# google-deepmind/bsuite

Hardware: AMD Instinct MI355X
Metric: env-steps/sec (higher is better)
Workload: dtype int32; 1 GPU; deep_sea/10 deep_sea {'size': 30, 'mapping_seed': 42} random actions, dense TimeStep; mode=e, lanes_per_gpu=1048576, global_lanes=1048576, episode_phases=staggered

## Files before the change

bsuite_amd/csrc/bsx_pair_device.h:

```cpp
#ifndef BSX_PAIR_DEVICE_H_
#define BSX_PAIR_DEVICE_H_

#include "bsx_device.h"
#include "bsx_policy.h"

template <class Fam, bool LEAN, bool NOMT>
__device__ __forceinline__ int bsx_fam_advance(const typename Fam::args& a, const typename Fam::shared& s, int64_t i, uint64_t lane,
                                               uint64_t step, int32_t st, int act, int32_t& nst, double& reward) {
  return Fam::template advance_nomt<LEAN, NOMT>(a, s, i, lane, step, st, act, nst, reward);
}

template <class Fam, bool LEAN = false, int MT = -1, int LPT = 1>
__device__ __forceinline__ void bsx_advance_body(const typename Fam::args& a, uint32_t block_id,
                                                 typename Fam::shared& s_fam, unsigned int* s_cnt,
                                                 int32_t* s_state = nullptr) {
  if (threadIdx.x < 2) s_cnt[threadIdx.x] = 0;
  Fam::stage(a, s_fam);
  __syncthreads();
  if constexpr (LPT == 2) {
    const uint64_t step = bsx_step_of(a.ctl);
    int64_t i[2];
    bool mine[2];
    int act[2], type[2] = {-1, -1};
    int32_t st[2];
// ... 145 lines not shown
      }
    }
  }
  if (mine) a.state[i] = st;
  bsx_pool_counts(a.ctl, n_last, n_first, s_cnt, block_id & (BSX_COUNTER_SHARDS - 1));
}

struct bsx_policy_args {
  const uint8_t* table;
  const int32_t* policy_index;
  int32_t* actions_out;
  double epsilon;
  uint64_t explore_seed;
  int32_t n_states, n_policies;
  uint32_t num_actions;
  int32_t in_lds;
};

template <class Fam, class HotFn>
__global__ void __launch_bounds__(BSX_BLOCK) bsx_policy_rollout_kernel(const typename Fam::args a, const int n_steps,
                                                                             int32_t* __restrict__ rows, const HotFn fn,
                                                                             const bsx_policy_args p) {
  __shared__ typename Fam::shared s_fam;
  __shared__ unsigned int s_cnt[2];
  __shared__ uint8_t s_tab[BSX_POLICY_LDS_BYTES];
  if (threadIdx.x < 2) s_cnt[threadIdx.x] = 0;
  Fam::stage(a, s_fam);
  const int S = p.n_states;
  const bool in_lds = p.in_lds != 0;
  if (in_lds) {
    for (int k = threadIdx.x; k < S; k += BSX_BLOCK) s_tab[k] = p.table[k];
  }
  __syncthreads();
  const int64_t B = a.ctl.n_lanes;
  const int64_t i = (int64_t)blockIdx.x * BSX_BLOCK + threadIdx.x;
  const bool mine = i < B;
  const uint64_t lane = a.ctl.lane_offset + (uint64_t)i;
  const uint64_t step0 = bsx_step_of(a.ctl);
  const bool explore = p.epsilon > 0.0;
  int32_t st = mine ? a.state[i] : 0;
  const uint8_t* __restrict__ tab = p.table;
  if (mine && p.policy_index != nullptr) tab += (int64_t)bsx_policy_clamp(p.policy_index[i], p.n_policies) * S;
  uint32_t n_last = 0, n_first = 0;
  uint32_t block_id = blockIdx.x;
#if defined(__HIP_DEVICE_COMPILE__)
  asm volatile("" : "+v"(block_id));
#endif
  if (mine) {
#pragma unroll 1
    for (int t = 0; t < n_steps; ++t) {
      const uint64_t step = step0 + (uint64_t)t;
      const int64_t oi = (int64_t)t * B + i;
      const int key = bsx_policy_clamp(fn.policy_key(st), S);
      uint32_t entry;
      if (in_lds) {
        entry = s_tab[key];
#if defined(__HIP_DEVICE_COMPILE__)
        asm volatile("" : "+v"(entry));
#endif
      } else {
        entry = tab[key];
      }
      uint32_t w0 = 0, w1 = 0, w2 = 0;
      if (explore) {
        const bsx_u32x4 w = bsx_policy_draws(p.explore_seed, lane, step);
        w0 = w.v[0]; w1 = w.v[1]; w2 = w.v[2];
      }
      const int act = bsx_policy_select(entry, Fam::resets(st), p.epsilon, w0, w1, w2, p.num_actions);
      int32_t nst; double reward;
      const int type = Fam::template advance<true>(a, s_fam, i, lane, step, st, act, nst, reward);
      st = nst;
      bsx_emit_at<0, 0, false, -1, BSX_OUT_SCALARS.rollout>(a.ctl, a.out, i, oi, lane, step, type, reward);
      bsx_index_store<BSX_OUT_INDEX.rollout>(rows, oi, nst, fn);
      bsx_st<BSX_OUT_SCALARS.rollout>(&p.actions_out[oi], (int32_t)act);
      n_last += type == BSX_LAST ? 1u : 0u;
      n_first += type == BSX_FIRST ? 1u : 0u;
    }
    a.state[i] = st;
  }
  bsx_pool_counts(a.ctl, n_last, n_first, s_cnt, block_id & (BSX_COUNTER_SHARDS - 1));
}

template <class Fam, class HotFn>
__device__ __forceinline__ void bsx_tab_eval_body(const typename Fam::args& a, const int n_steps, const HotFn& fn,
                                                  const bsx_policy_args& p, const bsx_policy_eval_t& out,
                                                  typename Fam::shared& s_fam, unsigned int* s_cnt, uint8_t* s_tab) {
  if (threadIdx.x < 2) s_cnt[threadIdx.x] = 0;
  Fam::stage(a, s_fam);
  const int S = p.n_states;
  const bool in_lds = p.in_lds != 0;
  if (in_lds) {
    for (int k = threadIdx.x; k < S; k += BSX_BLOCK) s_tab[k] = p.table[k];
  }
  __syncthreads();
  const int64_t i = (int64_t)blockIdx.x * BSX_BLOCK + threadIdx.x;
  const bool mine = i < a.ctl.n_lanes;
  const uint64_t lane = a.ctl.lane_offset + (uint64_t)i;
  const uint64_t step0 = bsx_step_of(a.ctl);
  const bool explore = p.epsilon > 0.0;
  uint32_t n_last = 0, n_first = 0;
  if (mine) {
    int32_t st = a.state[i];
    const uint8_t* __restrict__ tab = p.table;
    if (p.policy_index != nullptr) tab += (int64_t)bsx_policy_clamp(p.policy_index[i], p.n_policies) * S;
    bsx_eval_acc e = {0.0, 0.0, 0.0, 0};
    typename Fam::deferred pend = {};
#pragma unroll 1
    for (int t = 0; t < n_steps; ++t) {
      const uint64_t step = step0 + (uint64_t)t;
      const int key = bsx_policy_clamp(fn.policy_key(st), S);
      uint32_t entry;
      if (in_lds) {
        entry = s_tab[key];
#if defined(__HIP_DEVICE_COMPILE__)
        asm volatile("" : "+v"(entry));
#endif
      } else {
        entry = tab[key];
      }
      uint32_t w0 = 0, w1 = 0, w2 = 0;
      if (explore) {
        const bsx_u32x4 w = bsx_policy_draws(p.explore_seed, lane, step);
        w0 = w.v[0]; w1 = w.v[1]; w2 = w.v[2];
      }
      const int act = bsx_policy_select(entry, Fam::resets(st), p.epsilon, w0, w1, w2, p.num_actions);
      int32_t nst; double reward;
      const int type = Fam::advance_deferred(a, s_fam, i, lane, step, st, act, nst, reward, pend);
      st = nst;
      bsx_eval_accumulate(&e, type, reward);
      n_first += type == BSX_FIRST ? 1u : 0u;
    }
    n_last = (uint32_t)e.n;
    a.state[i] = st;
    out.episodes[i] = e.n;
    out.return_sum[i] = e.total;
    out.episode_return_sum[i] = e.done;
    Fam::commit_deferred(a, i, pend);
  }
  bsx_pool_counts(a.ctl, n_last, n_first, s_cnt, blockIdx.x);
}


template <class HotFn>
struct bsx_stream_seg {
  float* obs;
  const int32_t* state;
  int64_t n_lanes;
  uint32_t cells;
  uint32_t cells_magic;
  bsx_div64 dv;
  HotFn fn;
};

template <class HotFn, int K, int BS, bool NT = false>
__device__ __forceinline__ void bsx_hot_stream_body(float* __restrict__ obs,
                                                    const int32_t* __restrict__ state,
                                                    int64_t n_lanes, uint32_t cells,
                                                    uint32_t cells_magic, bsx_div64 dv,
                                                    const HotFn& fn, uint32_t block_id, int wave_contig = 1) {
  const uint64_t total = (uint64_t)n_lanes * cells;
  const uint64_t F0 = (uint64_t)block_id * (uint64_t)(K * 4 * BS);
  const uint64_t lane_b = __umul64hi(F0, dv.m) >> dv.s;
  const uint32_t r_b = (uint32_t)(F0 - lane_b * cells);
  const bool aligned = (cells & 3u) == 0;
  bsx_f4* __restrict__ o4 = reinterpret_cast<bsx_f4*>(obs + F0);
  const int32_t* __restrict__ st = state + lane_b;
  const uint64_t lanes_left = (uint64_t)n_lanes - lane_b;

  uint32_t dl[K];
  int r0[K];
  int32_t s0[K], s1[K];
  bool live[K];
#pragma unroll
  for (int u = 0; u < K; ++u) {
    const uint32_t c = wave_contig ? ((threadIdx.x >> 6) * (K * 64) + u * 64 + (threadIdx.x & 63))
                                   : (threadIdx.x + u * BS);
    const uint32_t f = r_b + (c << 2);
    dl[u] = __umulhi(f, cells_magic);
    r0[u] = (int)(f - dl[u] * cells);
    live[u] = F0 + ((uint64_t)c << 2) + 3 < total;
    s0[u] = live[u] ? st[dl[u]] : 0;
    s1[u] = (live[u] && !aligned && (uint64_t)dl[u] + 1 < lanes_left) ? st[dl[u] + 1] : 0;
  }
#pragma unroll
  for (int u = 0; u < K; ++u) {
    if (!live[u]) continue;
    int ha, hb;
    fn(s0[u], ha, hb);
    const int a0 = ha < 0 ? -1 : ha - r0[u], b0 = hb < 0 ? -1 : hb - r0[u];
    bsx_f4 v;
    v.x = (a0 == 0 || b0 == 0) ? 1.0f : 0.0f;
    v.y = (a0 == 1 || b0 == 1) ? 1.0f : 0.0f;
    v.z = (a0 == 2 || b0 == 2) ? 1.0f : 0.0f;
    v.w = (a0 == 3 || b0 == 3) ? 1.0f : 0.0f;
    const int over = (int)cells - r0[u];
    if (!aligned && over < 4) {
      int na, nb;
      fn(s1[u], na, nb);
      const int a1 = na < 0 ? -1 : na + over, b1 = nb < 0 ? -1 : nb + over;
      if (over <= 1) v.y = (a1 == 1 || b1 == 1) ? 1.0f : 0.0f;
      if (over <= 2) v.z = (a1 == 2 || b1 == 2) ? 1.0f : 0.0f;
      v.w = (a1 == 3 || b1 == 3) ? 1.0f : 0.0f;
    }
    {
      bsx_f4* dst = &o4[wave_contig ? ((threadIdx.x >> 6) * (K * 64) + u * 64 + (threadIdx.x & 63)) : (threadIdx.x + u * BS)];
      if (NT) __builtin_nontemporal_store(v, dst);
      else *dst = v;
    }
  }
  const uint64_t tail0 = total & ~3ull;
  if (tail0 != total && tail0 >= F0 && tail0 < F0 + (uint64_t)(K * 4 * BS) && threadIdx.x < 3) {
    const uint64_t F = tail0 + threadIdx.x;
    if (F < total) {
      const uint32_t f = r_b + (uint32_t)(F - F0);
      const uint32_t d = __umulhi(f, cells_magic);
      const int r = (int)(f - d * cells);
      int ha, hb;
      fn(st[d], ha, hb);
      obs[F] = (ha == r || hb == r) ? 1.0f : 0.0f;
    }
  }
}

template <class HotFn, int K, int BS>
__global__ void __launch_bounds__(BS) bsx_hot_stream_kernel(float* __restrict__ obs,
                                                                   const int32_t* __restrict__ state,
                                                                   int64_t n_lanes, uint32_t cells,
                                                                   uint32_t cells_magic, bsx_div64 dv,
                                                                   HotFn fn, int wave_contig) {
  bsx_hot_stream_body<HotFn, K, BS>(obs, state, n_lanes, cells, cells_magic, dv, fn, blockIdx.x, wave_contig);
}

template <class HotFn, int POLICY = BSX_ST_PLAIN>
__device__ __forceinline__ void bsx_tile_stream(float* __restrict__ tile, const int32_t* s_state, int lanes_here,
                                                uint32_t cells, uint32_t cells_magic, const HotFn& fn) {
  const uint32_t total = (uint32_t)lanes_here * cells;
  const uint32_t n_chunks = total >> 2;
  const bool aligned = (cells & 3u) == 0;
  bsx_f4* __restrict__ t4 = reinterpret_cast<bsx_f4*>(tile);
  for (uint32_t c = threadIdx.x; c < n_chunks; c += BSX_BLOCK) {
    const uint32_t f = c << 2;
    const uint32_t dl = bsx_div_cells(f, cells, cells_magic);
    const int r0 = (int)(f - dl * cells);
    int ha, hb;
    fn(s_state[dl], ha, hb);
    const int a0 = ha < 0 ? -1 : ha - r0, b0 = hb < 0 ? -1 : hb - r0;
    bsx_f4 v;
    v.x = (a0 == 0 || b0 == 0) ? 1.0f : 0.0f;
    v.y = (a0 == 1 || b0 == 1) ? 1.0f : 0.0f;
    v.z = (a0 == 2 || b0 == 2) ? 1.0f : 0.0f;
    v.w = (a0 == 3 || b0 == 3) ? 1.0f : 0.0f;
    const int over = (int)cells - r0;
    if (!aligned && over < 4) {
      int na, nb;
      fn(s_state[dl + 1], na, nb);
      const int a1 = na < 0 ? -1 : na + over, b1 = nb < 0 ? -1 : nb + over;
      if (over <= 1) v.y = (a1 == 1 || b1 == 1) ? 1.0f : 0.0f;
      if (over <= 2) v.z = (a1 == 2 || b1 == 2) ? 1.0f : 0.0f;
      v.w = (a1 == 3 || b1 == 3) ? 1.0f : 0.0f;
    }
    bsx_st<POLICY>(&t4[c], v);
  }
  const uint32_t f = (n_chunks << 2) + threadIdx.x;
  if (threadIdx.x < 3 && f < total) {
    const uint32_t dl = bsx_div_cells(f, cells, cells_magic);
    const int r = (int)(f - dl * cells);
    int ha, hb;
    fn(s_state[dl], ha, hb);
    tile[f] = (ha == r || hb == r) ? 1.0f : 0.0f;
  }
}

template <class Fam, bool LEAN, class HotFn>
__global__ void __launch_bounds__(BSX_BLOCK) bsx_fused_tile_kernel(const typename Fam::args a, float* __restrict__ obs,
                                                                   const uint32_t cells, const uint32_t cells_magic,
                                                                   const HotFn fn) {
  __shared__ typename Fam::shared s_fam;
  __shared__ unsigned int s_cnt[2];
  __shared__ int32_t s_state[BSX_BLOCK];
  bsx_advance_body<Fam, LEAN>(a, blockIdx.x, s_fam, s_cnt, s_state);
  const int64_t lane0 = (int64_t)blockIdx.x * BSX_BLOCK;
  const int64_t left = a.ctl.n_lanes - lane0;
  bsx_tile_stream<HotFn, BSX_ST_WT>(obs + lane0 * (int64_t)cells, s_state, left < BSX_BLOCK ? (int)left : BSX_BLOCK, cells, cells_magic, fn);
}

template <class Fam, bool LEAN, class HotFn>
__global__ void __launch_bounds__(BSX_BLOCK) bsx_fused_tile64_kernel(const typename Fam::args a, float* __restrict__ obs,
                                                                     const uint32_t cells, const uint32_t cells_magic,
                                                                     const HotFn fn) {
  __shared__ typename Fam::shared s_fam;
  __shared__ int32_t s_state[BSX_WAVE];
  Fam::stage(a, s_fam);
  __syncthreads();
  const int64_t lane0 = (int64_t)blockIdx.x * BSX_WAVE;
  const int64_t i = lane0 + threadIdx.x;
  int type = -1;
  if (threadIdx.x < BSX_WAVE && i < a.ctl.n_lanes) {
    const uint64_t lane = a.ctl.lane_offset + (uint64_t)i;
    const uint64_t step = bsx_step_of(a.ctl);
    int32_t nst; double reward;
    const int act = a.ctl.force_reset ? 0 : bsx_action(a.ctl, a.action, i, step);
    const int32_t st = a.ctl.state_in != nullptr ? a.ctl.state_in[i] : a.state[i];
    type = Fam::template advance<LEAN>(a, s_fam, i, lane, step, st, act, nst, reward);
    a.state[i] = nst;
    s_state[threadIdx.x] = nst;
    if (LEAN) bsx_emit_at<0, 0, false>(a.ctl, a.out, i, i, lane, step, type, reward);
    else bsx_emit(a.ctl, a.out, i, lane, step, type, reward);
  }
  if (threadIdx.x < BSX_WAVE && a.ctl.counters != nullptr) {
    const unsigned long long last = __ballot(type == BSX_LAST), first = __ballot(type == BSX_FIRST);
    if (threadIdx.x == 0 && (last | first) != 0ull) {
      unsigned long long* shard = (unsigned long long*)a.ctl.counters + (size_t)(blockIdx.x & (BSX_COUNTER_SHARDS - 1)) * BSX_COUNTER_STRIDE;
      if (last) atomicAdd(&shard[0], (unsigned long long)__popcll(last));
      if (first) atomicAdd(&shard[1], (unsigned long long)__popcll(first));
    }
  }
  __syncthreads();
  const int64_t left = a.ctl.n_lanes - lane0;
  bsx_tile_stream<HotFn, BSX_ST_WT>(obs + lane0 * (int64_t)cells, s_state, left < BSX_WAVE ? (int)left : BSX_WAVE, cells, cells_magic, fn);
}

template <class Fam, bool LEAN, class HotFn>
__global__ void __launch_bounds__(BSX_BLOCK) bsx_fused_rollout_kernel(const typename Fam::args a, const int n_steps,
                                                                      float* __restrict__ obs, const uint32_t cells,
                                                                      const uint32_t cells_magic, const HotFn fn) {
  __shared__ typename Fam::shared s_fam;
  __shared__ unsigned int s_cnt[2];
  __shared__ int32_t s_state[2][BSX_BLOCK];
  if (threadIdx.x < 2) s_cnt[threadIdx.x] = 0;
  Fam::stage(a, s_fam);
  __syncthreads();
  const int64_t B = a.ctl.n_lanes;
  const int64_t lane0 = (int64_t)blockIdx.x * BSX_BLOCK;
  const int64_t i = lane0 + threadIdx.x;
  const bool mine = i < B;
  const int lanes_here = B - lane0 < BSX_BLOCK ? (int)(B - lane0) : BSX_BLOCK;
  const uint64_t lane = a.ctl.lane_offset + (uint64_t)i;
  const uint64_t step0 = bsx_step_of(a.ctl);
  int32_t st = mine ? a.state[i] : 0;
  int act_next = mine ? a.action[i] : 0;
#pragma unroll 1
  for (int t = 0; t < n_steps; ++t) {
    int type = -1;
    const int act = act_next;
    if (mine) {
      if (t + 1 < n_steps) act_next = a.action[(int64_t)(t + 1) * B + i];
      int32_t nst; double reward;
      type = Fam::template advance<LEAN>(a, s_fam, i, lane, step0 + (uint64_t)t, st, act, nst, reward);
      st = nst;
      s_state[t & 1][threadIdx.x] = nst;
      if (LEAN) bsx_emit_at<0, 0, false>(a.ctl, a.out, i, (int64_t)t * B + i, lane, step0 + (uint64_t)t, type, reward);
      else bsx_emit_at(a.ctl, a.out, i, (int64_t)t * B + i, lane, step0 + (uint64_t)t, type, reward);
    }
    bsx_count_types(a.ctl, type, s_cnt);
    __syncthreads();
    bsx_tile_stream<HotFn, BSX_ST_NT>(obs + ((int64_t)t * B + lane0) * (int64_t)cells, s_state[t & 1], lanes_here, cells, cells_magic, fn);
  }
  if (mine) a.state[i] = st;
  bsx_final_barrier();
  bsx_flush_counts(a.ctl, s_cnt, blockIdx.x);
}

template <class Fam, bool LEAN, class HotFn, int K>
__global__ void __launch_bounds__(BSX_BLOCK) bsx_pipelined_kernel(const typename Fam::args a, const uint32_t adv_blocks,
// ... 163 lines not shown
```

bsuite_amd/csrc/bsx_pair_host.h:

```cpp
#ifndef BSX_PAIR_HOST_H_
#define BSX_PAIR_HOST_H_

#include "bsx_host.h"
#include "bsx_pair_device.h"

template <class Fam>
static inline int bsx_launch_advance(const typename Fam::args& a, hipStream_t st) {
  const int64_t blocks = bsx_blocks_of(a.ctl.n_lanes);
  if (blocks > 0x7FFFFFFF) return BSX_EINVAL;
  const bool lean = bsx_ctl_lean(a.ctl);
  static const int lpt2_min_blocks = bsx_env_int("BSX_ADVANCE_LPT2_MIN_BLOCKS", 4096);
  if (lean && lpt2_min_blocks > 0 && blocks >= lpt2_min_blocks) {
    bsx_advance2_kernel<Fam><<<dim3((unsigned)((blocks + 1) / 2)), dim3(BSX_BLOCK), 0, st>>>(a);
    return 0;
  }
  if (lean) bsx_advance_kernel<Fam, true><<<dim3((unsigned)blocks), dim3(BSX_BLOCK), 0, st>>>(a);
  else if (a.ctl.mt_state == nullptr) bsx_advance_kernel<Fam, false, 0><<<dim3((unsigned)blocks), dim3(BSX_BLOCK), 0, st>>>(a);
  else bsx_advance_kernel<Fam, false><<<dim3((unsigned)blocks), dim3(BSX_BLOCK), 0, st>>>(a);
  return 0;
}

void bsx_launch_pair_advance_delta(int32_t family, const void* args, const void* fn, int32_t* paint, uint32_t cells, int64_t blocks,
                                   hipStream_t st);

template <class Fam, class HotFn>
static inline int bsx_launch_advance_delta(const typename Fam::args& a, const HotFn& fn, int32_t* paint,
                                           uint32_t cells, hipStream_t st) {
  const int64_t blocks = bsx_blocks_of(a.ctl.n_lanes);
  if (blocks > 0x7FFFFFFF) return BSX_EINVAL;
  bsx_launch_pair_advance_delta(HotFn::FAMILY, &a, &fn, paint, cells, blocks, st);
  return 0;
}

int bsx_launch_hot_cells(float* obs, const int32_t* state, int64_t n_lanes, uint32_t cells, int32_t family, int32_t p0, int32_t p1,
                         hipStream_t st);

template <class HotFn, int K>
static inline int bsx_launch_hot_stream(float* obs, const int32_t* state, int64_t n_lanes, uint32_t cells,
                                        uint32_t cells_magic, HotFn fn, hipStream_t st) {
  const uint64_t total = (uint64_t)n_lanes * cells;
  if (cells < 4u || (reinterpret_cast<uintptr_t>(obs) & 15u) != 0)
    return bsx_launch_hot_cells(obs, state, n_lanes, cells, HotFn::FAMILY, fn.geom0(), fn.geom1(), st);
  const bsx_div64 dv = bsx_make_div64(cells);
  const uint64_t per_block = (uint64_t)K * 4 * BSX_BLOCK;
  const uint64_t blocks = (total + per_block - 1) / per_block;
  if (blocks > 0x7FFFFFFFull) return BSX_EINVAL;
  bsx_hot_stream_kernel<HotFn, K, BSX_BLOCK><<<dim3((unsigned)blocks), dim3(BSX_BLOCK), 0, st>>>(obs, state, n_lanes, cells, cells_magic, dv, fn, 1);
  return 0;
}

template <class HotFn, int K>
static inline int bsx_launch_narrow_stream(void* obs, const int32_t* state, int64_t n_lanes, uint32_t cells, int code,
                                           HotFn fn, hipStream_t st) {
  static const uint32_t one[4] = {0u, 0x01u, 0x3C00u, 0x3F80u};
  const int E = code == 1 ? 1 : 2, N = 16 / E;
  const uint64_t total = (uint64_t)n_lanes * cells;
  uint64_t head = ((16u - (reinterpret_cast<uintptr_t>(obs) & 15u)) & 15u) / (uint64_t)E;
  if (head > total) head = total;
  const uint64_t n_chunks = (total - head) / (uint64_t)N;
  const uint64_t per_block = (uint64_t)K * BSX_BLOCK;
  const uint64_t blocks = n_chunks == 0 ? 1 : (n_chunks + per_block - 1) / per_block;
  if (blocks > 0x7FFFFFFFull) return BSX_EINVAL;
  const bool wide = cells >= (uint32_t)N;
  const uint32_t magic = wide ? bsx_div_magic(cells) : 0u;
  const bsx_div64 dv = wide ? bsx_make_div64(cells) : bsx_div64{0, 0};
  const dim3 grid((unsigned)blocks), block(BSX_BLOCK);
  if (E == 1)
    bsx_narrow_stream_kernel<HotFn, 1, K><<<grid, block, 0, st>>>((uint8_t*)obs, state, n_lanes, cells, magic, dv,
                                                                   (uint32_t)head, n_chunks, one[code], fn);
  else
    bsx_narrow_stream_kernel<HotFn, 2, K><<<grid, block, 0, st>>>((uint8_t*)obs, state, n_lanes, cells, magic, dv,
                                                                   (uint32_t)head, n_chunks, one[code], fn);
  return 0;
}

template <class HotFn>
static inline bsx_stream_seg<HotFn> bsx_make_stream_seg(float* obs, const int32_t* state, int64_t n_lanes, uint32_t cells, const HotFn& fn) {
  bsx_stream_seg<HotFn> sg;
  sg.obs = obs; sg.state = state; sg.n_lanes = n_lanes; sg.cells = cells;
  sg.cells_magic = bsx_div_magic(cells); sg.dv = bsx_make_div64(cells); sg.fn = fn;
  return sg;
}

template <class Fam, class HotFn>
static inline int bsx_group_put_pair(bsx_group* g, int32_t index, const typename Fam::args& a, float* obs,
                                     int32_t* state, uint32_t cells, const HotFn& fn, int k) {
  if (cells < 4u) return BSX_ERANGE;
  memcpy(&g->args[(size_t)index * sizeof(typename Fam::args)], &a, sizeof(a));
  const bsx_stream_seg<HotFn> sg = bsx_make_stream_seg(obs, state, a.ctl.n_lanes, cells, fn);
  memcpy(&g->args2[(size_t)index * sizeof(sg)], &sg, sizeof(sg));
  const uint64_t b1 = (uint64_t)bsx_blocks_of(a.ctl.n_lanes);
  const uint64_t b2 = bsx_flat_blocks((uint64_t)a.ctl.n_lanes * cells, k);
  if (b1 > 0x3FFFFFFFull || b2 > 0x3FFFFFFFull) return BSX_EINVAL;
  g->blocks[index] = (int32_t)b1; g->blocks2[index] = (int32_t)b2;
  g->is_set[index] = 1;
  return 0;
}

void bsx_launch_pair_advance_group(int32_t family, const void* table, const bsx_group_index& gi, int64_t total_blocks, hipStream_t st);

template <class Fam, class HotFn, int K>
static int bsx_group_launch_pair(bsx_group* g, int phase, hipStream_t st) {
  if (phase != 1) bsx_launch_pair_advance_group(HotFn::FAMILY, g->d_args, g->index1(), g->total_blocks, st);
  if (phase != 0)
    bsx_hot_stream_group_kernel<HotFn, K><<<dim3((unsigned)g->total_blocks2), dim3(BSX_BLOCK), 0, st>>>(
        (const bsx_stream_seg<HotFn>*)g->d_args2, g->index2());
  return (int)hipGetLastError();
}

int bsx_launch_index_decode(int32_t* rows, const int32_t* state, int64_t n_lanes, int32_t family, int32_t p0, int32_t p1,
                            bool rollout, hipStream_t st);

static inline int bsx_check_policy_scalars(const bsx_call_t* call, const bsx_policy_t* pol, int32_t n_states) {
  if (call == nullptr || pol == nullptr) return BSX_ENULL;
  if ((call->flags & (BSX_CALL_OBS_MASK | BSX_CALL_OBS_INDEX)) != BSX_CALL_OBS_INDEX) return BSX_EMODE;
  if (call->logging != nullptr || call->wrap.kind != BSX_WRAP_NONE || call->stream.mt_state != nullptr ||
      call->stream.mt_pos != nullptr || call->reward_f64 != nullptr || call->obs_paint != nullptr ||
      call->state_alt != nullptr || call->action_ring > 1 || call->force_reset)
    return BSX_EMODE;
  if (call->n_steps < 1 || call->n_lanes < 0 || call->n_lanes > ((int64_t)1 << 40)) return BSX_EINVAL;
  if (pol->n_states != n_states || pol->n_policies < 1) return BSX_EINVAL;
  if (!(pol->epsilon >= 0.0 && pol->epsilon <= 1.0)) return BSX_ERANGE;
  return 0;
}

static inline int bsx_check_policy_call(const bsx_call_t* call, const bsx_policy_t* pol, int32_t n_states, const int32_t* state,
                                        const bsx_timestep_t& out, const double* info) {
  const int rc = bsx_check_policy_scalars(call, pol, n_states);
  if (rc != 0 || call->n_lanes == 0) return rc;
  if (pol->table == nullptr || pol->actions_out == nullptr || state == nullptr || info == nullptr ||
      out.reward == nullptr || out.discount == nullptr || out.step_type == nullptr || out.observation == nullptr)
    return BSX_ENULL;
  if (pol->n_policies > 1 && pol->policy_index == nullptr) return BSX_ENULL;
  if ((reinterpret_cast<uintptr_t>(out.observation) & 15u) != 0) return BSX_EALIGN;
  return 0;
}

static inline int bsx_check_policy_eval_call(const bsx_call_t* call, const bsx_policy_t* pol, int32_t n_states,
                                             const int32_t* state, const bsx_policy_eval_t& out, const double* info) {
  const int rc = bsx_check_policy_scalars(call, pol, n_states);
  if (rc != 0 || call->n_lanes == 0) return rc;
  if (pol->table == nullptr || state == nullptr || info == nullptr || out.episodes == nullptr || out.return_sum == nullptr ||
      out.episode_return_sum == nullptr)
    return BSX_ENULL;
  if (pol->n_policies > 1 && pol->policy_index == nullptr) return BSX_ENULL;
  if (call->action_ring < 0) return BSX_EINVAL;
  if (bsx_blocks_of(call->n_lanes) > 0x7FFFFFFF) return BSX_EINVAL;
  return 0;
}

static inline bsx_policy_args bsx_make_policy_args(const bsx_policy_t* pol, uint32_t num_actions) {
  bsx_policy_args p;
  p.table = pol->table;
  p.policy_index = pol->n_policies > 1 ? pol->policy_index : nullptr;
  p.actions_out = pol->actions_out;
  p.epsilon = pol->epsilon;
  p.explore_seed = pol->explore_seed;
  p.n_states = pol->n_states; p.n_policies = pol->n_policies;
  p.num_actions = num_actions;
  p.in_lds = (pol->n_policies == 1 && pol->n_states <= BSX_POLICY_LDS_BYTES) ? 1 : 0;
  return p;
}

template <class Fam, class HotFn>
static int bsx_policy_rollout_call(const typename Fam::args& a, const bsx_call_t* call, const bsx_policy_t* pol,
                                   uint32_t num_actions, bsx_timestep_t out, const HotFn& fn) {
// ... 122 lines not shown
```

bsuite_amd/csrc/deep_sea.hip:

```cpp
#include "bsx_pair_host.h"
#include "bsx_tab_eval.h"
#include "bsx_tab_sample_device.h"
#include "deep_sea_fam.h"
#include "pair_mixed.h"

template <int K>
__global__ void __launch_bounds__(BSX_BLOCK) deep_sea_step1_kernel(const deep_sea_fam::args a, const uint32_t cells,
                                                                   const uint32_t cells_magic, const bsx_div64 dv) {
  __shared__ deep_sea_fam::shared s_map[BSX_BLOCK / BSX_WAVE];
  const int wl = (int)(threadIdx.x & 63u);
  deep_sea_fam::shared& map = s_map[threadIdx.x >> 6];
  const int64_t n_lanes = a.ctl.n_lanes;
  const uint64_t step = bsx_step_of(a.ctl);
  const int32_t tag_new = (int32_t)(((uint32_t)(step + 1) & 1u) << DS_TAG_SHIFT);
  const bool forced = a.ctl.force_reset != 0;
  const deep_sea_hot fn{a.size};
  const uint64_t total = (uint64_t)n_lanes * cells;
  const uint64_t F0 = (uint64_t)blockIdx.x * (uint64_t)(K * 4 * BSX_BLOCK);
  const uint64_t lane_b = __umul64hi(F0, dv.m) >> dv.s;
  const uint32_t r_b = (uint32_t)(F0 - lane_b * cells);
  bsx_f4* __restrict__ o4 = reinterpret_cast<bsx_f4*>(a.out.observation + F0);
  const int32_t* __restrict__ st_b = a.state + lane_b;
  const int32_t* __restrict__ act_b = a.action + (forced ? 0 : lane_b);

  uint32_t dl[K];
  int r0[K];
  bool live[K];
#pragma unroll
  for (int u = 0; u < K; ++u) {
    const uint32_t c = (threadIdx.x >> 6) * (K * 64) + u * 64 + (threadIdx.x & 63);
    const uint32_t f = r_b + (c << 2);
    dl[u] = __umulhi(f, cells_magic);
    r0[u] = (int)(f - dl[u] * cells);
    live[u] = F0 + ((uint64_t)c << 2) + 3 < total;
  }
  const uint32_t dA = dl[0];
  uint32_t dB = dA;
  bool wrA = false, wrB = false;
#pragma unroll
  for (int u = 0; u < K; ++u) {
    if (live[u]) dB = dl[u];
  }
#pragma unroll
  for (int u = 0; u < K; ++u) {
    wrA |= live[u] && r0[u] == 0 && dl[u] == dA;
    wrB |= live[u] && r0[u] == 0 && dl[u] == dB && dB != dA;
  }
  const bool any = live[0];
  const int32_t wA = any ? st_b[dA] : 0, wB = any ? st_b[dB] : 0;
  const int aA = (any && !forced) ? act_b[dA] : 0, aB = (any && !forced) ? act_b[dB] : 0;

  const int map_words = (a.size * a.size + 31) >> 5;
  static_assert(DS_MAP_WORDS <= 2 * BSX_WAVE, "the per-wave copy of the action mapping is two passes at most");
  if (wl < map_words) map.map[wl] = a.mapping_bits[wl];
  if (wl + BSX_WAVE < map_words) map.map[wl + BSX_WAVE] = a.mapping_bits[wl + BSX_WAVE];
  bsx_wave_sync();


  auto resolve = [&](uint32_t d, int32_t w, int act, bool writer, int& type) -> int32_t {
    type = -1;
    if (!writer && (w & DS_TAG_BIT) == tag_new) return w;
    const int64_t L = (int64_t)lane_b + d;
    int32_t nst; double reward;
    const int ty = deep_sea_fam::advance<true, 1>(a, map, L, a.ctl.lane_offset + (uint64_t)L, step, w, act, nst, reward, writer);
    if (writer) {
      type = ty;
      a.state[L] = nst;
      bsx_emit_at<0, 0, false>(a.ctl, a.out, L, L, a.ctl.lane_offset + (uint64_t)L, step, ty, reward);
    }
    return nst;
  };
  int tA = -1, tB = -1;
  int32_t nA = 0, nB = 0;
  if (any) {
    nA = resolve(dA, wA, aA, wrA, tA);
    nB = dB != dA ? resolve(dB, wB, aB, wrB, tB) : nA;
  }
  int hA, hB, unused;
  fn(nA, hA, unused);
  fn(nB, hB, unused);
#pragma unroll
  for (int u = 0; u < K; ++u) {
    if (!live[u]) continue;
    int hot = dl[u] == dA ? hA : hB;
    const int p0 = hot < 0 ? -1 : hot - r0[u];
    bsx_f4 v;
    v.x = p0 == 0 ? 1.0f : 0.0f;
    v.y = p0 == 1 ? 1.0f : 0.0f;
    v.z = p0 == 2 ? 1.0f : 0.0f;
    v.w = p0 == 3 ? 1.0f : 0.0f;
    o4[(threadIdx.x >> 6) * (K * 64) + u * 64 + (threadIdx.x & 63)] = v;
  }
  const unsigned int n_last = (unsigned int)__popcll(__ballot(tA == BSX_LAST)) + (unsigned int)__popcll(__ballot(tB == BSX_LAST));
  const unsigned int n_first = (unsigned int)__popcll(__ballot(tA == BSX_FIRST)) + (unsigned int)__popcll(__ballot(tB == BSX_FIRST));
  if (a.ctl.counters != nullptr && wl == 0 && (n_last | n_first) != 0u) {
    unsigned long long* shard = (unsigned long long*)a.ctl.counters +
                                (size_t)((blockIdx.x * (BSX_BLOCK / BSX_WAVE) + (threadIdx.x >> 6)) & (BSX_COUNTER_SHARDS - 1)) * BSX_COUNTER_STRIDE;
    if (n_last) atomicAdd(&shard[0], (unsigned long long)n_last);
    if (n_first) atomicAdd(&shard[1], (unsigned long long)n_first);
  }
}

static int deep_sea_check_cfg(const bsx_deep_sea_t* cfg) {
  return (cfg->size < 1 || cfg->size > BSX_DEEP_SEA_MAX_SIZE) ? BSX_ERANGE : 0;
}

static void deep_sea_fill(const bsx_deep_sea_t* cfg, const bsx_call_t* call, const int32_t* action, int32_t* state,
                          bsx_timestep_t out, double* info, deep_sea_fam::args* a) {
  a->ctl = bsx_make_ctl(call);
  a->action = action; a->state = state; a->out = out; a->info = info;
  a->move_cost = cfg->move_cost; a->inv_size = cfg->inv_size;
  a->size = cfg->size; a->deterministic = cfg->deterministic;
  for (int w = 0; w < DS_MAP_WORDS; ++w) a->mapping_bits[w] = cfg->mapping_bits[w];
}

static int deep_sea_make(const bsx_deep_sea_t* cfg, const bsx_call_t* call, const int32_t* action,
                         int32_t* state, bsx_timestep_t out, double* info, deep_sea_fam::args* a) {
  if (cfg == nullptr) return BSX_ENULL;
  int rc = bsx_check_call(call, action, out, true, true);
  if (rc != 0) return rc;
  if ((rc = deep_sea_check_cfg(cfg)) != 0) return rc;
  if (call->stream.mt_state != nullptr && !cfg->deterministic && call->stream.mt_gauss == nullptr)
    return BSX_ENULL;
  if (call->n_lanes > 0 && (state == nullptr || info == nullptr)) return BSX_ENULL;
  deep_sea_fill(cfg, call, action, state, out, info, a);
  return 0;
}

extern "C" int bsx_deep_sea_step(const bsx_deep_sea_t* cfg, const bsx_call_t* call,
                                 const int32_t* action, int32_t* state, bsx_timestep_t out,
                                 double* info) {
  deep_sea_fam::args a;
  int rc = deep_sea_make(cfg, call, action, state, out, info, &a);
  if (rc != 0) return rc;
  if (call->n_lanes == 0) return 0;
  const uint32_t cells = (uint32_t)(cfg->size * cfg->size);
  static const int step1_env = bsx_env_int("BSX_DEEP_SEA_STEP1", 1);
  if (step1_env != 0 && (int64_t)call->n_lanes * cells * 4 <= ((int64_t)1 << 30) && (call->flags & BSX_CALL_STATE_TAGGED) && call->n_steps <= 1 && call->action_ring <= 1 && cfg->deterministic && bsx_ctl_lean(a.ctl) &&
      call->obs_paint == nullptr && bsx_call_obs(call) == 0 && !bsx_call_index(call) && (cells & 3u) == 0 && cells >= 3u * 256u) {
    constexpr int K = 4;
    const uint64_t total = (uint64_t)call->n_lanes * cells;
    const uint64_t blocks = (total + (uint64_t)K * 4 * BSX_BLOCK - 1) / ((uint64_t)K * 4 * BSX_BLOCK);
    if (blocks > 0x7FFFFFFFull) return BSX_EINVAL;
    deep_sea_step1_kernel<K><<<dim3((unsigned)blocks), dim3(BSX_BLOCK), 0, (hipStream_t)call->hip_stream>>>(
        a, cells, bsx_div_magic(cells), bsx_make_div64(cells));
    return bsx_launch_status();
  }
  return bsx_pair_call<deep_sea_fam, deep_sea_hot, 4>(a, call, action, state, out, cells, deep_sea_hot{cfg->size});
}

extern "C" int bsx_deep_sea_policy_rollout(const bsx_deep_sea_t* cfg, const bsx_call_t* call, const bsx_policy_t* policy,
                                           int32_t* state, bsx_timestep_t out, double* info) {
  if (cfg == nullptr || call == nullptr || policy == nullptr) return BSX_ENULL;
  int rc = deep_sea_check_cfg(cfg);
  if (rc == 0) rc = bsx_check_policy_call(call, policy, bsx_policy_states_deep_sea(cfg->size), state, out, info);
  if (rc != 0 || call->n_lanes == 0) return rc;
  deep_sea_fam::args a;
  rc = deep_sea_make(cfg, call, policy->actions_out, state, out, info, &a);
  if (rc != 0) return rc;
  a.action = nullptr;
  return bsx_policy_rollout_call<deep_sea_fam, deep_sea_hot>(a, call, policy, 2u, out, deep_sea_hot{cfg->size});
}

extern "C" int bsx_deep_sea_policy_evaluate(const bsx_deep_sea_t* cfg, const bsx_call_t* call, const bsx_policy_t* policy,
                                             int32_t* state, bsx_policy_eval_t out, double* info) {
  if (cfg == nullptr || call == nullptr || policy == nullptr) return BSX_ENULL;
  int rc = deep_sea_check_cfg(cfg);
  if (rc == 0) rc = bsx_check_policy_eval_call(call, policy, bsx_policy_states_deep_sea(cfg->size), state, out, info);
  if (rc != 0 || call->n_lanes == 0) return rc;
  bsx_tab_eval_args e;
  deep_sea_fill(cfg, call, nullptr, state, bsx_timestep_t{}, info, &e.fam.deep_sea);
  return bsx_tab_eval_call(e, BSX_FAM_DEEP_SEA, call, policy, 2u, out);
}

extern "C" int bsx_deep_sea_policy_sample(const bsx_deep_sea_t* cfg, const bsx_call_t* call, const bsx_policy_logits_t* policy,
                                          int32_t* state, bsx_timestep_t out, double* info) {
  if (cfg == nullptr || call == nullptr || policy == nullptr) return BSX_ENULL;
  int rc = deep_sea_check_cfg(cfg);
  if (rc == 0) rc = bsx_check_tab_softmax_call(call, policy, bsx_policy_states_deep_sea(cfg->size), 2, state, out, info);
  if (rc != 0 || call->n_lanes == 0) return rc;
  bsx_tab_softmax_args s;
  rc = deep_sea_make(cfg, call, policy->actions_out, state, out, info, &s.fam.deep_sea);
  if (rc != 0) return rc;
  s.fam.deep_sea.action = nullptr;
  return bsx_tab_softmax_call(s, BSX_FAM_DEEP_SEA, call, policy, true, reinterpret_cast<int32_t*>(out.observation), bsx_policy_eval_t{});
}

extern "C" int bsx_deep_sea_policy_sample_evaluate(const bsx_deep_sea_t* cfg, const bsx_call_t* call,
                                                   const bsx_policy_logits_t* policy, int32_t* state, bsx_policy_eval_t out,
                                                   double* info) {
  if (cfg == nullptr || call == nullptr || policy == nullptr) return BSX_ENULL;
  int rc = deep_sea_check_cfg(cfg);
  if (rc == 0) rc = bsx_check_tab_softmax_eval_call(call, policy, bsx_policy_states_deep_sea(cfg->size), 2, state, out, info);
  if (rc != 0 || call->n_lanes == 0) return rc;
  bsx_tab_softmax_args s;
  deep_sea_fill(cfg, call, nullptr, state, bsx_timestep_t{}, info, &s.fam.deep_sea);
  return bsx_tab_softmax_call(s, BSX_FAM_DEEP_SEA, call, policy, false, nullptr, out);
}

extern "C" int bsx_group_set_deep_sea(bsx_group_t* g, int32_t index, const bsx_deep_sea_t* cfg,
                                      const bsx_call_t* call, const int32_t* action, int32_t* state,
                                      bsx_timestep_t out, double* info) {
  if (g == nullptr) return BSX_ENULL;
  if (call != nullptr && (bsx_call_obs(call) != 0 || bsx_call_index(call))) return BSX_EMODE;
  int rc;
  deep_sea_fam::args a;
  if (bsx_is_mixed_pair_group(g)) {
    rc = deep_sea_make(cfg, call, action, state, out, info, &a);
    if (rc != 0) return rc;
    a.ctl.state_in = call->state_alt;
    const uint32_t cells = (uint32_t)(cfg->size * cfg->size);
    if (cells < 4u) return BSX_ERANGE;
    const bsx_stream_seg<deep_sea_hot> sg = bsx_make_stream_seg(out.observation, state, a.ctl.n_lanes, cells, deep_sea_hot{cfg->size});
    return bsx_mixed_put(g, BSX_FAM_DEEP_SEA, index, call, &a, sizeof(a), &sg, sizeof(sg),
                              (uint64_t)bsx_blocks_of(a.ctl.n_lanes),
                              bsx_flat_blocks((uint64_t)a.ctl.n_lanes * cells, PAIR_DEEP_SEA_K), 0);
  }
  rc = bsx_group_check_set(g, BSX_FAM_DEEP_SEA, index, call, sizeof(deep_sea_fam::args),
                           sizeof(bsx_stream_seg<deep_sea_hot>), 0);
  if (rc != 0) return rc;
  rc = deep_sea_make(cfg, call, action, state, out, info, &a);
  if (rc != 0) return rc;
  g->launch = bsx_group_launch_pair<deep_sea_fam, deep_sea_hot, 4>;
  g->n_phases = 2;
  return bsx_group_put_pair<deep_sea_fam, deep_sea_hot>(g, index, a, out.observation, state,
                                                        (uint32_t)(cfg->size * cfg->size), deep_sea_hot{cfg->size}, 4);
}
```

bsuite_amd/csrc/deep_sea_fam.h:

```cpp
#ifndef BSX_DEEP_SEA_FAM_H_
#define BSX_DEEP_SEA_FAM_H_

#include "bsx_device.h"
#include "bsx_policy.h"

#define DS_RESET_BIT (1 << 17)
#define DS_TAG_SHIFT 18
#define DS_TAG_BIT (1 << DS_TAG_SHIFT)
#define DS_MAP_WORDS (BSX_DEEP_SEA_MAX_SIZE * BSX_DEEP_SEA_MAX_SIZE / 32)

struct deep_sea_fam {
  struct args {
    bsx_ctl ctl;
    const int32_t* action;
    int32_t* state;
    bsx_timestep_t out;
    double* info;
    double move_cost;
    double inv_size;
    int32_t size;
    int32_t deterministic;
    uint32_t mapping_bits[DS_MAP_WORDS];
  };
  struct shared { uint32_t map[DS_MAP_WORDS]; };

  __device__ static __forceinline__ void stage(const args& a, shared& s) {
    const int map_words = (a.size * a.size + 31) >> 5;
    for (int w = threadIdx.x; w < map_words; w += BSX_BLOCK) s.map[w] = a.mapping_bits[w];
  }

  template <bool LEAN = false, int DET = -1, bool NOMT = false>
  __device__ static __forceinline__ int advance(const args& a, const shared& s, int64_t i, uint64_t lane,
                                                uint64_t step, int32_t st, int act, int32_t& nst,
                                                double& reward, const bool commit = true) {
    BSX_NO_CONTRACT
    const int N = a.size;
    const bool deterministic = DET == 1 || a.deterministic;
    int row = st & 0xFF, col = (st >> 8) & 0xFF, bad = (st >> 16) & 1;
    int type;
    reward = 0.0;
    if (a.ctl.force_reset || (st & DS_RESET_BIT)) {
      row = 0; col = 0; bad = 0;
      type = BSX_FIRST;
    } else {
      const int cell = row * N + col;
      const int mapped = (int)((s.map[cell >> 5] >> (cell & 31)) & 1u);
      const bool right = (act == mapped);
      bsx_draws d;
      bsx_draws_begin<(LEAN || NOMT) ? 0 : -1>(&d, a.ctl, i, lane, step);
      if (col == N - 1 && right) {
        reward += 1.0;
        if (commit) a.info[a.ctl.n_lanes + i] += 1.0;
      }
      if (!deterministic && row == N - 1 && (col == 0 || col == N - 1))
        reward += bsx_normal(&d);
      if (right) {
        bool moves = true;
        if (!deterministic || (!LEAN && !NOMT && a.ctl.mt_state != nullptr)) {
          const double u = bsx_uniform(&d);
          moves = (u > a.inv_size) || deterministic;
        }
        if (moves) col = col + 1 > N - 1 ? N - 1 : col + 1;
        reward -= a.move_cost;
      } else {
        if (row == col) bad = 1;
        col = col - 1 < 0 ? 0 : col - 1;
      }
      bsx_draws_end<(LEAN || NOMT) ? 0 : -1>(&d, a.ctl, i);
      row += 1;
      if (row == N) {
        if (bad && commit) a.info[i] += 1.0;
        type = BSX_LAST;
      } else {
        type = BSX_MID;
      }
    }
    nst = row | (col << 8) | (bad << 16) | (type == BSX_LAST ? DS_RESET_BIT : 0) | (int32_t)(((uint32_t)(step + 1) & 1u) << DS_TAG_SHIFT);
    return type;
  }
  template <bool LEAN, bool NOMT>
  __device__ static __forceinline__ int advance_nomt(const args& a, const shared& s, int64_t i, uint64_t lane, uint64_t step,
                                                     int32_t st, int act, int32_t& nst, double& reward) {
    return advance<LEAN, -1, NOMT>(a, s, i, lane, step, st, act, nst, reward);
  }
  __device__ static __forceinline__ bool resets(int32_t st) { return (st & DS_RESET_BIT) != 0; }

  struct deferred { uint32_t bad, good; };
  __device__ static __forceinline__ int advance_deferred(const args& a, const shared& s, int64_t i, uint64_t lane, uint64_t step,
                                                         int32_t st, int act, int32_t& nst, double& reward, deferred& d) {
    const int type = advance<true>(a, s, i, lane, step, st, act, nst, reward, false);
    if (type != BSX_FIRST) {
      const int col = (st >> 8) & 0xFF, cell = (st & 0xFF) * a.size + col;
      const int mapped = (int)((s.map[cell >> 5] >> (cell & 31)) & 1u);
      d.good += (col == a.size - 1 && act == mapped) ? 1u : 0u;
      d.bad += (type == BSX_LAST && ((nst >> 16) & 1) != 0) ? 1u : 0u;
    }
    return type;
  }
  __device__ static __forceinline__ void commit_deferred(const args& a, int64_t i, const deferred& d) {
    if (d.bad != 0u) a.info[i] += (double)d.bad;
    if (d.good != 0u) a.info[a.ctl.n_lanes + i] += (double)d.good;
  }
};

struct deep_sea_hot {
  int N;
  static constexpr int INDEX_K = 1;
  static constexpr int FAMILY = BSX_FAM_DEEP_SEA;
  int geom0() const { return N; }
  int geom1() const { return 0; }
  __device__ __forceinline__ void operator()(int32_t st, int& a, int& b) const {
    const int row = st & 0xFF, col = (st >> 8) & 0xFF;
    a = row < N ? row * N + col : -1;
    b = -1;
  }
  __device__ __forceinline__ int policy_key(int32_t st) const {
    int a, b;
    (*this)(st, a, b);
    return bsx_policy_key_deep_sea(a);
  }
};

#endif
```

bsuite_amd/environments/deep_sea.py:

```python
import warnings
from typing import Optional

import numpy as np
import torch

from bsuite_amd import _native
from bsuite_amd.environments import base

NUM_EPISODES = 10000


class DeepSea(base.Environment):

  _info_keys = ('total_bad_episodes', 'denoised_return')
  _info_int_keys = ('total_bad_episodes',)

  def __init__(self,
               size: int,
               deterministic: bool = True,
               unscaled_move_cost: float = 0.01,
               randomize_actions: bool = True,
               seed: Optional[int] = None,
               mapping_seed: Optional[int] = None,
               **engine_kwargs):
    if not 1 <= size <= _native.DEEP_SEA_MAX_SIZE:
      raise ValueError(f'size must be in [1, {_native.DEEP_SEA_MAX_SIZE}]')
    super().__init__(obs_shape=(size, size), num_actions=2, seed=seed, **engine_kwargs)
    self._size = size
    self._deterministic = deterministic
    self._unscaled_move_cost = unscaled_move_cost

    if randomize_actions:
      self._mapping_rng = np.random.RandomState(mapping_seed)
      self._action_mapping = self._mapping_rng.binomial(1, 0.5, [size, size])
    else:
      warnings.warn('Environment is in debug mode (randomize_actions=False).'
                    'Only randomized_actions=True is the DeepSea environment.')
      self._action_mapping = np.ones([size, size])

    if not self._deterministic:
      optimal_no_cost = (1 - 1 / self._size) ** (self._size - 1)
    else:
      optimal_no_cost = 1.
    self._optimal_return = optimal_no_cost - self._unscaled_move_cost

    cfg = _native.DeepSeaCfg()
    cfg.size = size
    cfg.deterministic = int(bool(deterministic))
    cfg.move_cost = float(unscaled_move_cost) / size
    cfg.inv_size = 1 / size
    flat = np.asarray(self._action_mapping).reshape(-1) == 1
    for idx in np.nonzero(flat)[0]:
      cfg.mapping_bits[int(idx) >> 5] |= (1 << (int(idx) & 31))
    self._cfg = cfg
    self.bsuite_num_episodes = NUM_EPISODES

  def _state_tensors(self):
    return dict(state=torch.full((self._batch,), 1 << 17, dtype=torch.int32, device=self._device))

  _abi_name = 'deep_sea'
  _supports_delta = True
  _supports_narrow_obs = True
  _index_width = 1
  _pipelined_rollout = True

  _state_tag_bit = 1 << 18
  _state_lib_bits = 1 << 18

  _policy_abi = 'bsx_deep_sea_policy_rollout'
  _policy_eval_abi = 'bsx_deep_sea_policy_evaluate'
  _policy_sample_abi = 'bsx_deep_sea_policy_sample'
  _policy_sample_eval_abi = 'bsx_deep_sea_policy_sample_evaluate'

  @property
  def policy_num_states(self) -> int:
    return self._size * self._size

  @property
  def optimal_return(self):
    return self._optimal_return
```

Measured before the change: 1.758 billion env-steps/s.

## Fuse deep_sea advance and observation stream into one beside-launch kernel

Adds a combined kernel where some blocks advance lane state while other blocks paint the one-hot observation by resolving the next position themselves from the old state and action. It is used for large boards above a byte threshold. This avoids a separate launch and the serial dependency between advance and observation painting. The state word now caches the mapping bit of the next cell so resolving blocks usually skip the global mapping lookup. The cost is redundant state transition work and extra action reads in the stream blocks.

```diff
diff --git a/bsuite_amd/csrc/bsx_pair_device.h b/bsuite_amd/csrc/bsx_pair_device.h
--- a/bsuite_amd/csrc/bsx_pair_device.h
+++ b/bsuite_amd/csrc/bsx_pair_device.h
@@ -321,25 +321,30 @@
   HotFn fn;
 };
 
-template <class HotFn, int K, int BS, bool NT = false>
+struct bsx_no_resolve { static constexpr bool ACTIVE = false; };
+template <class HotFn, int K, int BS, bool NT = false, class Resolve = bsx_no_resolve>
 __device__ __forceinline__ void bsx_hot_stream_body(float* __restrict__ obs,
                                                     const int32_t* __restrict__ state,
                                                     int64_t n_lanes, uint32_t cells,
                                                     uint32_t cells_magic, bsx_div64 dv,
-                                                    const HotFn& fn, uint32_t block_id, int wave_contig = 1) {
+                                                    const HotFn& fn, uint32_t block_id, int wave_contig = 1,
+                                                    const Resolve& rs = Resolve()) {
   const uint64_t total = (uint64_t)n_lanes * cells;
   const uint64_t F0 = (uint64_t)block_id * (uint64_t)(K * 4 * BS);
   const uint64_t lane_b = __umul64hi(F0, dv.m) >> dv.s;
   const uint32_t r_b = (uint32_t)(F0 - lane_b * cells);
-  const bool aligned = (cells & 3u) == 0;
+  const bool aligned = Resolve::ACTIVE || (cells & 3u) == 0;
   bsx_f4* __restrict__ o4 = reinterpret_cast<bsx_f4*>(obs + F0);
   const int32_t* __restrict__ st = state + lane_b;
   const uint64_t lanes_left = (uint64_t)n_lanes - lane_b;
+  const int32_t* __restrict__ xc = nullptr;
+  if constexpr (Resolve::ACTIVE) xc = rs.column != nullptr ? rs.column + lane_b : nullptr;
 
   uint32_t dl[K];
   int r0[K];
   int32_t s0[K], s1[K];
   bool live[K];
+  (void)xc;
 #pragma unroll
   for (int u = 0; u < K; ++u) {
     const uint32_t c = wave_contig ? ((threadIdx.x >> 6) * (K * 64) + u * 64 + (threadIdx.x & 63))
@@ -355,7 +360,8 @@
   for (int u = 0; u < K; ++u) {
     if (!live[u]) continue;
     int ha, hb;
-    fn(s0[u], ha, hb);
+    if constexpr (Resolve::ACTIVE) rs.hot(s0[u], xc, dl[u], ha, hb);
+    else fn(s0[u], ha, hb);
     const int a0 = ha < 0 ? -1 : ha - r0[u], b0 = hb < 0 ? -1 : hb - r0[u];
     bsx_f4 v;
     v.x = (a0 == 0 || b0 == 0) ? 1.0f : 0.0f;
@@ -378,7 +384,7 @@
     }
   }
   const uint64_t tail0 = total & ~3ull;
-  if (tail0 != total && tail0 >= F0 && tail0 < F0 + (uint64_t)(K * 4 * BS) && threadIdx.x < 3) {
+  if (!Resolve::ACTIVE && tail0 != total && tail0 >= F0 && tail0 < F0 + (uint64_t)(K * 4 * BS) && threadIdx.x < 3) {
     const uint64_t F = tail0 + threadIdx.x;
     if (F < total) {
       const uint32_t f = r_b + (uint32_t)(F - F0);
diff --git a/bsuite_amd/csrc/bsx_pair_host.h b/bsuite_amd/csrc/bsx_pair_host.h
--- a/bsuite_amd/csrc/bsx_pair_host.h
+++ b/bsuite_amd/csrc/bsx_pair_host.h
@@ -3,6 +3,11 @@
 
 #include "bsx_host.h"
 #include "bsx_pair_device.h"
+
+template <class Fam>
+static inline void bsx_launch_advance2(const typename Fam::args& a, unsigned grid, hipStream_t st) {
+  bsx_advance2_kernel<Fam><<<dim3(grid), dim3(BSX_BLOCK), 0, st>>>(a);
+}
 
 template <class Fam>
 static inline int bsx_launch_advance(const typename Fam::args& a, hipStream_t st) {
@@ -11,7 +16,7 @@
   const bool lean = bsx_ctl_lean(a.ctl);
   static const int lpt2_min_blocks = bsx_env_int("BSX_ADVANCE_LPT2_MIN_BLOCKS", 4096);
   if (lean && lpt2_min_blocks > 0 && blocks >= lpt2_min_blocks) {
-    bsx_advance2_kernel<Fam><<<dim3((unsigned)((blocks + 1) / 2)), dim3(BSX_BLOCK), 0, st>>>(a);
+    bsx_launch_advance2<Fam>(a, (unsigned)((blocks + 1) / 2), st);
     return 0;
   }
   if (lean) bsx_advance_kernel<Fam, true><<<dim3((unsigned)blocks), dim3(BSX_BLOCK), 0, st>>>(a);
diff --git a/bsuite_amd/csrc/deep_sea.hip b/bsuite_amd/csrc/deep_sea.hip
--- a/bsuite_amd/csrc/deep_sea.hip
+++ b/bsuite_amd/csrc/deep_sea.hip
@@ -101,6 +101,69 @@
   }
 }
 
+struct deep_sea_beside_resolve {
+  static constexpr bool ACTIVE = true;
+  const deep_sea_fam::args& a;
+  const int32_t* column;
+  int32_t tag_new;
+  __device__ __forceinline__ void hot(int32_t w, const int32_t* __restrict__ act_b, uint32_t d, int& ha, int& hb) const {
+    const int N = a.size;
+    int row = w & 0xFF, col = (w >> 8) & 0xFF;
+    if ((w & DS_TAG_BIT) != tag_new) {
+      if (a.ctl.force_reset || (w & DS_RESET_BIT)) {
+        row = 0; col = 0;
+      } else {
+        int mapped = (w >> DS_MAP_SHIFT) & 1;
+        if ((((w >> DS_MAP_SHIFT) ^ (w >> (DS_MAP_SHIFT + 1))) & 1) == 0) {
+          const int cell = row * N + col;
+          mapped = (int)((a.mapping_bits[(cell >> 5) & (DS_MAP_WORDS - 1)] >> (cell & 31)) & 1u);
+        }
+        if (act_b[d] == mapped) col = col + 1 > N - 1 ? N - 1 : col + 1;
+        else col = col - 1 < 0 ? 0 : col - 1;
+        row += 1;
+      }
+    }
+    ha = row < N ? row * N + col : -1;
+    hb = -1;
+  }
+};
+static_assert((DS_MAP_WORDS & (DS_MAP_WORDS - 1)) == 0, "deep_sea_beside_resolve masks the mapping word's index");
+
+template <int K, int LPT>
+__global__ void __launch_bounds__(BSX_BLOCK) bsx_deep_sea_beside_kernel(const deep_sea_fam::args a, const uint32_t adv_blocks,
+                                                                        const uint32_t cells, const uint32_t cells_magic,
+                                                                        const bsx_div64 dv) {
+  __shared__ deep_sea_fam::shared s_fam;
+  __shared__ unsigned int s_cnt[2];
+  const bsx_pipe_role r = bsx_pipe_role_of(blockIdx.x, gridDim.x, adv_blocks, 0u);
+  if (r.adv) {
+    bsx_advance_body<deep_sea_fam, true, -1, LPT>(a, r.index, s_fam, s_cnt);
+    return;
+  }
+  const deep_sea_beside_resolve rs{a, a.ctl.force_reset ? nullptr : a.action,
+                                   (int32_t)(((uint32_t)(bsx_step_of(a.ctl) + 1) & 1u) << DS_TAG_SHIFT)};
+  bsx_hot_stream_body<deep_sea_hot, K, BSX_BLOCK, false, deep_sea_beside_resolve>(
+      a.out.observation, a.state, a.ctl.n_lanes, cells, cells_magic, dv, deep_sea_hot{a.size}, r.index, 1, rs);
+}
+
+constexpr int DS_BESIDE_LPT = 2;
+
+template <>
+void bsx_launch_advance2<deep_sea_fam>(const deep_sea_fam::args& a, unsigned grid, hipStream_t st) {
+  bsx_deep_sea_beside_kernel<4, DS_BESIDE_LPT><<<dim3(grid), dim3(BSX_BLOCK), 0, st>>>(a, grid, 0u, 0u, bsx_div64{0, 0});
+}
+
+static int deep_sea_launch_beside(const deep_sea_fam::args& a, const bsx_call_t* call, uint32_t cells) {
+  constexpr int K = 4, LPT = DS_BESIDE_LPT;
+  const uint64_t adv_lanes = (uint64_t)LPT * BSX_BLOCK;
+  const uint64_t adv_blocks = ((uint64_t)call->n_lanes + adv_lanes - 1) / adv_lanes;
+  const uint64_t str_blocks = bsx_flat_blocks((uint64_t)call->n_lanes * cells, K);
+  if (adv_blocks + str_blocks > 0x7FFFFFFFull) return BSX_EINVAL;
+  bsx_deep_sea_beside_kernel<K, LPT><<<dim3((unsigned)(adv_blocks + str_blocks)), dim3(BSX_BLOCK), 0, (hipStream_t)call->hip_stream>>>(
+      a, (uint32_t)adv_blocks, cells, bsx_div_magic(cells), bsx_make_div64(cells));
+  return bsx_launch_status();
+}
+
 static int deep_sea_check_cfg(const bsx_deep_sea_t* cfg) {
   return (cfg->size < 1 || cfg->size > BSX_DEEP_SEA_MAX_SIZE) ? BSX_ERANGE : 0;
 }
@@ -136,8 +199,14 @@
   if (call->n_lanes == 0) return 0;
   const uint32_t cells = (uint32_t)(cfg->size * cfg->size);
   static const int step1_env = bsx_env_int("BSX_DEEP_SEA_STEP1", 1);
-  if (step1_env != 0 && (int64_t)call->n_lanes * cells * 4 <= ((int64_t)1 << 30) && (call->flags & BSX_CALL_STATE_TAGGED) && call->n_steps <= 1 && call->action_ring <= 1 && cfg->deterministic && bsx_ctl_lean(a.ctl) &&
-      call->obs_paint == nullptr && bsx_call_obs(call) == 0 && !bsx_call_index(call) && (cells & 3u) == 0 && cells >= 3u * 256u) {
+  static const int beside_min_bytes = bsx_env_int("BSX_DEEP_SEA_BESIDE_MIN_BYTES", 1 << 30);
+  const int64_t board_bytes = (int64_t)call->n_lanes * cells * 4;
+  const bool one_launch = (call->flags & BSX_CALL_STATE_TAGGED) && call->n_steps <= 1 && call->action_ring <= 1 && cfg->deterministic && bsx_ctl_lean(a.ctl) &&
+      call->obs_paint == nullptr && bsx_call_obs(call) == 0 && !bsx_call_index(call) && (cells & 3u) == 0 && cells >= 3u * 256u;
+  if (one_launch && beside_min_bytes >= 0 && board_bytes > (int64_t)beside_min_bytes) {
+    return deep_sea_launch_beside(a, call, cells);
+  }
+  if (step1_env != 0 && board_bytes <= ((int64_t)1 << 30) && one_launch) {
     constexpr int K = 4;
     const uint64_t total = (uint64_t)call->n_lanes * cells;
     const uint64_t blocks = (total + (uint64_t)K * 4 * BSX_BLOCK - 1) / ((uint64_t)K * 4 * BSX_BLOCK);
diff --git a/bsuite_amd/csrc/deep_sea_fam.h b/bsuite_amd/csrc/deep_sea_fam.h
--- a/bsuite_amd/csrc/deep_sea_fam.h
+++ b/bsuite_amd/csrc/deep_sea_fam.h
@@ -7,6 +7,9 @@
 #define DS_RESET_BIT (1 << 17)
 #define DS_TAG_SHIFT 18
 #define DS_TAG_BIT (1 << DS_TAG_SHIFT)
+#define DS_MAP_SHIFT 19
+#define DS_MAP_BIT (1 << DS_MAP_SHIFT)
+#define DS_NOMAP_BIT (1 << (DS_MAP_SHIFT + 1))
 #define DS_MAP_WORDS (BSX_DEEP_SEA_MAX_SIZE * BSX_DEEP_SEA_MAX_SIZE / 32)
 
 struct deep_sea_fam {
@@ -75,7 +78,10 @@
         type = BSX_MID;
       }
     }
-    nst = row | (col << 8) | (bad << 16) | (type == BSX_LAST ? DS_RESET_BIT : 0) | (int32_t)(((uint32_t)(step + 1) & 1u) << DS_TAG_SHIFT);
+    const int ncell = row < N ? row * N + col : 0;
+    const bool nmap = row < N && ((s.map[ncell >> 5] >> (ncell & 31)) & 1u) != 0u;
+    nst = row | (col << 8) | (bad << 16) | (type == BSX_LAST ? DS_RESET_BIT : 0) | (int32_t)(((uint32_t)(step + 1) & 1u) << DS_TAG_SHIFT) |
+          (nmap ? DS_MAP_BIT : DS_NOMAP_BIT);
     return type;
   }
   template <bool LEAN, bool NOMT>
diff --git a/bsuite_amd/environments/deep_sea.py b/bsuite_amd/environments/deep_sea.py
--- a/bsuite_amd/environments/deep_sea.py
+++ b/bsuite_amd/environments/deep_sea.py
@@ -65,7 +65,7 @@
   _pipelined_rollout = True
 
   _state_tag_bit = 1 << 18
-  _state_lib_bits = 1 << 18
+  _state_lib_bits = 7 << 18
 
   _policy_abi = 'bsx_deep_sea_policy_rollout'
   _policy_eval_abi = 'bsx_deep_sea_policy_evaluate'
```

After: 1.755 billion env-steps/s. About the same (-0.2%).
